# Fatlonder/tinyfusers

Hardware: AMD Instinct MI355X
Metric: unet_denoise_steps_per_sec (higher is better)
Workload: dtype f16; 1 GPU; SD1.5 UNet single denoise step (CFG batch 2 + DDIM update), 64x64x4 latent, 1 image per GPU, fp16 conv/linear, 50-step DDIM schedule; global_batch=1, parallelism=dp1 (batch-sharded, RCCL weight broadcast only, no per-step collective), launch=hipGraph

## Files before the change

### include/tinyfusers_hip.h

```cpp
#ifndef TINYFUSERS_HIP_H
#define TINYFUSERS_HIP_H
#include <stddef.h>
#include <stdint.h>
#ifdef __cplusplus
extern "C" {
#endif

typedef struct tfStream_st* tfStream_t;
typedef struct tfEvent_st* tfEvent_t;
typedef struct tfGraph_st* tfGraph_t;
typedef struct tfComm_st* tfComm_t;
typedef struct tfFunction_st* tfFunction_t;

#define TF_OK 0
#define TF_E_ARG 10001
#define TF_E_UNSUPPORTED 10002
#define TF_E_WORKSPACE 10003
#define TF_E_STATE 10004

#define TF_MEMCPY_H2D 1
#define TF_MEMCPY_D2H 2
#define TF_MEMCPY_D2D 3

int tf_init(int device);
// ... 203 lines not shown
                       void* workspace, size_t workspace_bytes, const void* x3, const void* x4, int C3, int C4, void* gn_partial,
                       size_t gn_partial_bytes, int gn_groups, int* gn_chunks, tfStream_t s);
int tf_conv2d_fused_norm_16(int dtype, void* y, const void* x, const void* x2, const void* w, const void* bias, const void* bias_nc, long long bias_nc_stride,
                            const void* residual, int N, int H, int W, int C1, int C2, int Cout, int R, int S, int stride, int pad, int upsample,
                            void* workspace, size_t workspace_bytes, const void* x3, const void* x4, int C3, int C4, void* gn_partial,
                            size_t gn_partial_bytes, int gn_groups, int* gn_chunks, void* z, const void* z_gamma, const void* z_beta, float z_eps,
                            int z_silu, int* z_written, tfStream_t s);
int tf_conv2d_gn_16(int dtype, void* y, const void* x, const void* x2, const void* w, const void* bias, const void* bias_nc, long long bias_nc_stride,
                    const void* residual, int N, int H, int W, int C1, int C2, int Cout, int R, int S, int stride, int pad, int upsample,
                    void* workspace, size_t workspace_bytes, const void* x3, const void* x4, int C3, int C4, void* gn_partial,
                    size_t gn_partial_bytes, int gn_groups, int* gn_chunks, const void* in_gamma, const void* in_beta, const void* in_partial,
                    int in_chunks, int in_groups1, const void* in_partial2, int in_chunks2, int in_groups2, int in_groups, float in_eps, int in_silu,
                    tfStream_t s);
int tf_linear_16(int dtype, void* y, const void* x, const void* w, const void* bias, const void* residual, int M, int N, int K, int act,
                 void* workspace, size_t workspace_bytes, tfStream_t s);
int tf_ln_fold_weights_16(int dtype, void* w_out, void* bias_out, void* colsum_out_f32, const void* w, const void* bias, const void* gamma, const void* beta,
                          int N, int K, tfStream_t s);
int tf_linear_ln_16(int dtype, void* y, const void* x, const void* w_folded, const void* bias_folded, const void* colsum_f32, const void* residual,
                    int M, int N, int K, int act, float eps, tfStream_t s);
int tf_gemv_16(int dtype, void* y, const void* x, const void* w, const void* bias, int M, int N, int K, int silu_input, tfStream_t s);
int tf_sdpa_16(int dtype, void* o, const void* q, const void* k, const void* v, int B, int NH, int Tq, int Tk, int HS,
               long long q_sb, long long q_sh, long long q_st, long long k_sb, long long k_sh, long long k_st,
               long long v_sb, long long v_sh, long long v_st, long long o_sb, long long o_sh, long long o_st, int causal, tfStream_t s);
int tf_group_norm_apply_16(int dtype, void* y, const void* x, const void* gamma, const void* beta, const void* partial, int chunks,
                           int N, int HW, int C, int G, float eps, int silu, tfStream_t s);
int tf_group_norm_apply_cat_16(int dtype, void* y, const void* x, const void* x2, const void* gamma, const void* beta, const void* partial, int chunks,
                               int groups1, const void* partial2, int chunks2, int groups2, int N, int HW, int C1, int C2, int G, float eps,
                               int silu, tfStream_t s);
int tf_add_16(int dtype, void* y, const void* a, const void* b, long long n, tfStream_t s);

int tf_silu_f16(void* y, const void* x, long long n, tfStream_t s);
int tf_sigmoid_f16(void* y, const void* x, long long n, tfStream_t s);
int tf_gelu_f16(void* y, const void* x, long long n, tfStream_t s);
int tf_quick_gelu_f16(void* y, const void* x, long long n, tfStream_t s);
int tf_embedding_f16(void* out, const void* table, const void* ids, const void* pos, long long n_tokens, int dim, int vocab,
                     int T, tfStream_t s);
int tf_debug_nonfinite(const void* x, long long nbytes, int is_f32, void* flag, tfStream_t s);
int tf_debug_checksum(const void* x, long long nbytes, void* sum, tfStream_t s);
int tf_geglu_f16(void* y, const void* x, int rows, int C, tfStream_t s);
int tf_add_f16(void* y, const void* a, const void* b, long long n, tfStream_t s);
int tf_add_bias_nc_f16(void* y, const void* x, const void* bias_nc, int N, int HW, int C, tfStream_t s);
int tf_upsample2x_nhwc_f16(void* y, const void* x, int N, int H, int W, int C, tfStream_t s);
int tf_concat_channels_f16(void* y, const void* a, const void* b, long long rows, int Ca, int Cb, tfStream_t s);
int tf_im2col_nhwc_f16(void* y, const void* x, int N, int H, int W, int C, int R, int S, int stride, int pad, int Kpad, tfStream_t s);
int tf_im2col_rows_nhwc_f16(void* y, const void* x, int N, int H, int W, int C, int R, int S, int stride, int pad, int Kpad, int ho_begin, int ho_end,
                            tfStream_t s);
// ... 64 lines not shown
```

### tinyfusers_amd/attention/attention.py

```python
import numpy as np

from .. import config
from ..ff.group_norm import GroupNorm
from ..ff.layer_norm import LayerNorm
from ..ff.linear import Linear, fold_layer_norm, linear_f16, linear_ln_f16
from ..ff.nn import FeedForward
from ..native import hip
from ..storage.tensor import DeviceArray, _sh, is_bfloat16
from ..vision.conv2d import Conv2d, _conv
from .sdpa import sdpa_dual_strided, sdpa_strided


def _concat_rows(ws):
    k = ws[0].shape[1]
    n = sum(w.shape[0] for w in ws)
    out = DeviceArray.empty((n, k), ws[0].dtype, "row")
    off = 0
    for w in ws:
        hip.tf_memcpy_async(out.ptr + off, w.ptr, w.nbytes, 3, _sh())
        off += w.nbytes
    return out


class AttnBlock:

    def __init__(self, in_channels, init=True):
        self.norm = GroupNorm(32, in_channels, init=init)
        self.q = Conv2d(in_channels, in_channels, kernel_size=[1, 1], init=init)
        self.k = Conv2d(in_channels, in_channels, kernel_size=[1, 1], init=init)
        self.v = Conv2d(in_channels, in_channels, kernel_size=[1, 1], init=init)
        self.proj_out = Conv2d(in_channels, in_channels, kernel_size=[1, 1], init=init)

    def __call__(self, x):
# ... 21 lines not shown
class CrossAttention:
    def __init__(self, query_dim, context_dim, n_heads, d_head, init=True):
        self.to_q = Linear(query_dim, n_heads * d_head, bias=False, init=init)
        self.to_k = Linear(context_dim, n_heads * d_head, bias=False, init=init)
        self.to_v = Linear(context_dim, n_heads * d_head, bias=False, init=init)
        self.num_heads = n_heads
        self.head_size = d_head
        self.to_out = [Linear(n_heads * d_head, query_dim, init=init)]
        self._fused = None

    def _fused_weights(self, self_attn):
        key = (self.to_q.weight.wkey, self.to_k.weight.wkey, self.to_v.weight.wkey, self_attn)
        if self._fused is None or self._fused[0] != key:
            ws = [self.to_q.weight, self.to_k.weight, self.to_v.weight] if self_attn else [self.to_k.weight, self.to_v.weight]
            self._fused = (key, _concat_rows(ws))
        return self._fused[1]

    def _folded(self, ln, self_attn):
        w = self._fused_weights(True) if self_attn else self.to_q.weight
        key = (w.wkey, ln.weight.wkey, ln.bias.wkey)
        if getattr(self, "_ln_fold", None) is None or self._ln_fold[0] != key:
            self._ln_fold = (key, fold_layer_norm(w, None, ln))
        return self._ln_fold[1]

    def project_kv(self, context):
        return linear_f16(context, self._fused_weights(False))

    def __call__(self, x, context=None, residual=None, kv=None, ln=None, ip=None):
        if ip is not None and context is None and kv is None:
            raise ValueError("CrossAttention: ip= is for cross-attention (context= or kv=), not self-attention")
        b, t, _ = x.shape
        nh, hs = self.num_heads, self.head_size
        c = nh * hs
        from ..ff import fp8
        mx_in = fp8.ATTENTION and ln is not None and fp8.linear_ok(b * t, 3 * c if (context is None and kv is None) else c, x.shape[-1])
        if mx_in:
            if getattr(self, "_cache8", None) is None:
                self._cache8 = {"qkv": {}, "q": {}, "out": {}}
            x8 = fp8.layer_norm_mx(x, ln)
        if context is None and kv is None:
            if mx_in:
                w8, wsc = fp8.pack_weight(self._fused_weights(True), self._cache8["qkv"])
                qkv = fp8.linear_mx(x8, w8, wsc, None)
            elif ln is not None:
                qkv = linear_ln_f16(x, self._folded(ln, True), ln.eps)
            else:
                qkv = linear_f16(x, self._fused_weights(True))
            q, k, v = qkv, qkv.view((b, t, 3 * c), "row", c), qkv.view((b, t, 3 * c), "row", 2 * c)
            tk, qs, ks = t, (t * 3 * c, hs, 3 * c), (t * 3 * c, hs, 3 * c)
        else:
            if mx_in:
                w8, wsc = fp8.pack_weight(self.to_q.weight, self._cache8["q"])
                q = fp8.linear_mx(x8, w8, wsc, None)
            else:
                q = linear_ln_f16(x, self._folded(ln, False), ln.eps) if ln is not None else linear_f16(x, self.to_q.weight)
            if kv is None:
                kv = self.project_kv(context)
            if hasattr(kv, "ld"):
                tk, ld = kv.arr.shape[1], kv.ld
                k = kv.arr.view(kv.arr.shape, "row", kv.off)
                v = kv.arr.view(kv.arr.shape, "row", kv.off + c)
            else:
                tk, ld = kv.shape[1], 2 * c
                k, v = kv, kv.view(kv.shape, "row", c)
            qs, ks = (t * c, hs, c), (tk * ld, hs, ld)
        o = DeviceArray.empty((b, t, c), x.dtype, "row")
        if config.head_merge == "reference_exact":
            os_ = (nh * t * hs, t * hs, hs)
        else:
            os_ = (t * c, hs, c)
        if ip is None:
            sdpa_strided(o, q, k, v, b, nh, t, tk, hs, qs, ks, ks, os_)
        else:
            kv2, scale_ptr = ip
            if kv2.arr.ndim != 3 or kv2.arr.shape[0] != b or kv2.c != c or kv2.off + 2 * c > kv2.ld:
                raise ValueError(f"CrossAttention: ip K|V {kv2.arr.shape} (columns {kv2.off} .. {kv2.off + 2 * c} of {kv2.ld}) does not fit a batch of {b} with {c} channels")
            tk2 = kv2.arr.shape[1]
            k2s = (tk2 * kv2.ld, hs, kv2.ld)
            sdpa_dual_strided(o, q, k, v, kv2.arr.view(kv2.arr.shape, "row", kv2.off), kv2.arr.view(kv2.arr.shape, "row", kv2.off + c), scale_ptr,
                              b, nh, t, tk, tk2, hs, qs, ks, ks, k2s, k2s, os_)
        lo = self.to_out[0]
        if fp8.ATTENTION and fp8.linear_ok(b * t, lo.weight.shape[0], c):
            if getattr(self, "_cache8", None) is None:
                self._cache8 = {"qkv": {}, "q": {}, "out": {}}
            w8, wsc = fp8.pack_weight(lo.weight, self._cache8["out"])
            return fp8.linear_mx(fp8.quantize_mx(o), w8, wsc, lo.bias, residual=residual)
        return lo(o, residual=residual)


class BasicTransformerBlock:
    def __init__(self, dim, context_dim, n_heads, d_head, init=True):
        self.attn1 = CrossAttention(dim, dim, n_heads, d_head, init=init)
        self.ff = FeedForward(dim, init=init)
        self.attn2 = CrossAttention(dim, context_dim, n_heads, d_head, init=init)
# ... 109 lines not shown
```

### tinyfusers_amd/attention/sdpa.py

```python
import numpy as np

from ..native import check, hip, lib
from ..storage.tensor import DeviceArray, _sh, dtag


def sdpa_strided(o, q, k, v, B, NH, Tq, Tk, HS, qs, ks, vs, os_, causal=False):
    assert dtag(q.dtype) == dtag(k.dtype) == dtag(v.dtype) == dtag(o.dtype), "sdpa: q / k / v / o must hold the same 16-bit type"
    hip.tf_sdpa_16(dtag(q.dtype), o.ptr, q.ptr, k.ptr, v.ptr, B, NH, Tq, Tk, HS, *qs, *ks, *vs, *os_, 1 if causal else 0, _sh())
    return o


SDPA_INSTANCES = {1: "generic", 2: "dma16", 3: "dma32", 4: "dma32_w8", 5: "split"}


def sdpa_instance(dtype, B, NH, Tq, Tk, HS, k_st=None, v_st=None, causal=False):
    k_st, v_st = HS if k_st is None else k_st, HS if v_st is None else v_st
    rc = lib.tf_sdpa_instance(dtag(dtype), B, NH, Tq, Tk, HS, k_st, v_st, 1 if causal else 0)
    if rc not in SDPA_INSTANCES:
        check(rc, "tf_sdpa_instance")
    return SDPA_INSTANCES[rc]


def sdpa_dual_strided(o, q, k, v, k2, v2, scale_ptr, B, NH, Tq, Tk, Tk2, HS, qs, ks, vs, k2s, v2s, os_):
    assert dtag(q.dtype) == dtag(k.dtype) == dtag(v.dtype) == dtag(k2.dtype) == dtag(v2.dtype) == dtag(o.dtype), "sdpa_dual: q / k / v / k2 / v2 / o must hold the same 16-bit type"
    hip.tf_sdpa_dual_16(dtag(q.dtype), o.ptr, q.ptr, k.ptr, v.ptr, Tk, k2.ptr, v2.ptr, Tk2, scale_ptr, B, NH, Tq, HS, *qs, *ks, *vs, *k2s, *v2s, *os_, _sh())
    return o


def sdpa_dual_instance(dtype, B, NH, Tq, Tk, Tk2, HS, k_st=None, v_st=None, k2_st=None, v2_st=None):
    st = [HS if s is None else s for s in (k_st, v_st, k2_st, v2_st)]
    rc = lib.tf_sdpa_dual_instance(dtag(dtype), B, NH, Tq, Tk, Tk2, HS, *st)
    if rc not in SDPA_INSTANCES:
        check(rc, "tf_sdpa_dual_instance")
    return SDPA_INSTANCES[rc]


def _is_causal_mask(m, tq, tk):
    m = np.asarray(m)
    if m.shape[-2:] != (tq, tk):
        return False
    m2 = m.reshape(-1, tq, tk)[0]
    tri = np.tril(np.ones((tq, tk), dtype=bool))
    if m.dtype == np.bool_:
        return bool((m2 == tri).all())
    return bool(np.isneginf(m2[~tri]).all() and (m2[tri] == 0).all())


def _additive_mask(attn_mask, B, NH, Tq, Tk):
    m = np.asarray(attn_mask.numpy() if isinstance(attn_mask, DeviceArray) else attn_mask)
    if m.dtype == np.bool_:
        m = np.where(m, np.float32(0.0), np.float32(-np.inf))
    m = m.astype(np.float32)
    if m.ndim < 2 or m.shape[-2:] != (Tq, Tk):
        m = np.broadcast_to(m, (Tq, Tk)) if m.ndim <= 2 else np.broadcast_to(m, m.shape[:-2] + (Tq, Tk))
    if m.ndim > 2 and int(np.prod(m.shape[:-2])) > 1:
        m = np.broadcast_to(m, (B, NH, Tq, Tk)).reshape(B * NH * Tq, Tk)
    else:
# ... 52 lines not shown
```

### tinyfusers_amd/build.py

```python
import concurrent.futures as cf
import os
import subprocess
import sys

HERE = os.path.dirname(os.path.abspath(__file__))
CSRC = os.path.join(HERE, "csrc")
LIBDIR = os.path.join(HERE, "lib")
LIB = os.path.join(LIBDIR, "libtinyfusers_hip.so")
LIB_ABLATION = os.path.join(LIBDIR, "libtinyfusers_hip_ablation.so")
LIB_ASAN = os.path.join(LIBDIR, "libtinyfusers_hip_asan.so")
ASAN_FLAGS = ["-fsanitize=address,undefined", "-fno-gpu-sanitize", "-fno-omit-frame-pointer", "-g", "-fno-sanitize-recover=undefined"]
SOURCES = ["gemm_k_pp16.hip", "gemm_k_pp16_bf16.hip", "gemm_k_pp8.hip", "gemm_k_igemm_128.hip", "gemm_k_igemm_128_bf16.hip", "gemm_k_igemm_64.hip", "gemm_k_igemm_64_bf16.hip",
           "gemm_k_igemm_160.hip", "gemm_k_igemm_160_bf16.hip", "gemm_k_patch.hip", "gemm_k_patch_bf16.hip", "sdpa.hip", "sdpa_bf16.hip", "sdpa_split.hip", "sdpa_split_bf16.hip",
           "sdpa_dual.hip", "sdpa_dual_bf16.hip", "gemm_k_igemm8.hip", "gemm_k_c4.hip", "gemm_k_c4_bf16.hip", "gemm_k_c8.hip", "gemm_k_c8_bf16.hip", "gemm_k_ar.hip", "gemm_k_ar_bf16.hip", "gemm_k_pp3.hip", "gemm_k_pp3_bf16.hip", "gemm.hip", "gemm_reduce.hip", "norm.hip", "elementwise.hip", "runtime.hip", "sgemm.hip",
           "comm.hip", "rtc.hip", "sampler.hip", "img2img.hip", "control.hip", "lora.hip", "vit.hip", "freeu.hip"]
FLAGS = ["--offload-arch=gfx950", "-O3", "-fPIC", "-std=c++17", "-Wall", "-Wno-unused-function", "-ffp-contract=fast"]
SDPA_UNITS = ["sdpa.hip", "sdpa_bf16.hip", "sdpa_split.hip", "sdpa_split_bf16.hip", "sdpa_dual.hip", "sdpa_dual_bf16.hip"]
EXTRA = {s: ["-mllvm", "-amdgpu-mfma-vgpr-form", "-fno-honor-nans"] for s in SDPA_UNITS}


def _hipcc():
    for c in (os.environ.get("HIPCC"), "/opt/rocm/bin/hipcc", "hipcc"):
        if c and (os.path.isabs(c) and os.path.exists(c) or not os.path.isabs(c)):
            return c
    raise RuntimeError("hipcc not found")


def _stale(target, deps):
    if not os.path.exists(target):
        return True
    t = os.path.getmtime(target)
    return any(os.path.getmtime(d) > t for d in deps)


def sanitizer_env(base=None):
    import glob
# ... 40 lines not shown
```

### tinyfusers_amd/config.py

```python
import os


def _flag(name, default):
    v = os.environ.get(name)
    return default if v is None else v not in ("0", "", "false", "False")


head_merge = "reference_exact"

fuse_layer_norm = _flag("TF_FUSE_LAYER_NORM", True)

parallel_branches = _flag("TF_PARALLEL_BRANCHES", False)

fold_skip_projection = _flag("TF_FOLD_SKIP", True)

fold_proj_out = _flag("TF_FOLD_PROJ_OUT", True)

concat_stats = _flag("TF_CONCAT_STATS", True)
concat_stats_max_elems = int(os.environ.get("TF_CONCAT_STATS_MAX_ELEMS", str(4 << 20)))

fuse_group_norm = _flag("TF_FUSE_GROUP_NORM", True)
fuse_group_norm_max_elems = int(os.environ.get("TF_FUSE_GROUP_NORM_MAX_ELEMS", str(4 << 20)))
fuse_group_norm_3x3 = _flag("TF_FUSE_GROUP_NORM_3X3", False)

fuse_reduce_norm = _flag("TF_FUSE_REDUCE_NORM", True)

cfg_parallel = _flag("TF_CFG_PARALLEL", False)

hoist_step_invariants = _flag("TF_HOIST_STEP_INVARIANTS", True)

dtype = "fp16"


def set_dtype(name):
    global dtype
    if name not in ("fp16", "fp8", "bf16"):
        raise ValueError(f"config.set_dtype: unknown dtype {name!r}")
    if name == "bf16" and (parallel_branches or cfg_parallel):
        raise ValueError("config.set_dtype('bf16'): not with TF_PARALLEL_BRANCHES / TF_CFG_PARALLEL (fp16-only experiments)")
# ... 6 lines not shown
```

### tinyfusers_amd/csrc/gemm.hip

```cpp
#include "gemm_prof.h"

__global__ void __launch_bounds__(256) k_quantize_fp8(unsigned char* __restrict__ y, const half_t* __restrict__ x, float scale, long long n8) {
  long long gs = (long long)gridDim.x * 256;
  for (long long i = (long long)blockIdx.x * 256 + threadIdx.x; i < n8; i += gs) {
    h8 v = *reinterpret_cast<const h8*>(x + i * 8);
    f4 a, b;
    for (int e = 0; e < 4; ++e) { a[e] = (float)v[e] * scale; b[e] = (float)v[4 + e] * scale; }
    *reinterpret_cast<uint2*>(y + i * 8) = pack8_fp8(a, b);
  }
}
__global__ void __launch_bounds__(256) k_quantize_mx8(unsigned char* __restrict__ y, const half_t* __restrict__ x, long long rows, int C) {
  const long long n8 = rows * (C >> 3), gs = (long long)gridDim.x * 256;
  const int cv8 = C >> 3;
  for (long long i0 = (long long)blockIdx.x * 256; i0 < n8; i0 += gs) {
    const long long i = i0 + threadIdx.x;
    const bool live = i < n8;
    f4 a = {0.f, 0.f, 0.f, 0.f}, b = {0.f, 0.f, 0.f, 0.f};
    if (live) {
      h8 v = *reinterpret_cast<const h8*>(x + i * 8);
      for (int e = 0; e < 4; ++e) { a[e] = (float)v[e]; b[e] = (float)v[4 + e]; }
    }
    unsigned sb;
    const uint2 code = mx_quant8(a, b, sb);
    if (live) {
// ... 608 lines not shown
int tf_ln_fold_weights_f16(void* w_out, void* bias_out, void* colsum_out, const void* w, const void* bias, const void* gamma, const void* beta,
                           int N, int K, tfStream_t s) {
  return tf_ln_fold_weights_16(TF_DTYPE_F16, w_out, bias_out, colsum_out, w, bias, gamma, beta, N, K, s);
}

int tf_linear_ln_16(int dtype, void* y, const void* x, const void* w_folded, const void* bias_folded, const void* colsum, const void* residual, int M, int N,
                    int K, int act, float eps, tfStream_t s) {
  TF_REQUIRE_DTYPE("tf_linear_ln_16");
  TF_REQUIRE(bias_folded && colsum, "tf_linear_ln_f16: null tensor");
  TF_REQUIRE(K >= 64 && K % 64 == 0, "tf_linear_ln_f16: K=%d must be a positive multiple of 64", K);
  TF_REQUIRE((act == 1 ? N % 16 == 0 : N % 4 == 0), "tf_linear_ln_f16: N=%d must be a multiple of 4 (16 for GEGLU)", N);
  GemmP p;
  int rc = linear_problem(p, "tf_linear_ln_f16", EL_16, y, x, w_folded, bias_folded, residual, M, N, K, act);
  if (rc || M == 0) return rc;
  p.ln_colsum = (const float*)colsum; p.ln_eps = eps;
  p.bf16 = dtype == TF_DTYPE_BF16;
  return run_forced(p, nullptr, 0, s);
}
int tf_linear_ln_f16(void* y, const void* x, const void* w_folded, const void* bias_folded, const void* colsum, const void* residual, int M, int N,
                     int K, int act, float eps, tfStream_t s) {
  return tf_linear_ln_16(TF_DTYPE_F16, y, x, w_folded, bias_folded, colsum, residual, M, N, K, act, eps, s);
}

int tf_gemv_16(int dtype, void* y, const void* x, const void* w, const void* bias, int M, int N, int K, int silu_input, tfStream_t s) {
  TF_REQUIRE_DTYPE("tf_gemv_16");
  TF_REQUIRE(y && x && w && M >= 1 && M <= 8 && N >= 1 && K % 8 == 0, "tf_gemv_f16: needs 1 <= M <= 8 (M=%d) and K %% 8 == 0 (K=%d)", M, K);
  if (dtype == TF_DTYPE_BF16) hipLaunchKernelGGL(k_gemv<true>, dim3(ceil_div(N, 4)), dim3(256), 0, tf_hs(s), (half_t*)y, (const half_t*)x, (const half_t*)w, (const half_t*)bias, M, N, K, silu_input);
  else hipLaunchKernelGGL(k_gemv<false>, dim3(ceil_div(N, 4)), dim3(256), 0, tf_hs(s), (half_t*)y, (const half_t*)x, (const half_t*)w, (const half_t*)bias, M, N, K, silu_input);
  TF_LAUNCH_CHECK();
  return TF_OK;
}
int tf_gemv_f16(void* y, const void* x, const void* w, const void* bias, int M, int N, int K, int silu_input, tfStream_t s) {
  return tf_gemv_16(TF_DTYPE_F16, y, x, w, bias, M, N, K, silu_input, s);
}

}
```

### tinyfusers_amd/csrc/gemm_family.h

```cpp
#pragma once
#include "gemm_reduce.h"

enum Variant {
  V_NONE = -1,
  V_RING = 0,
  V_WIDE = 1,
  V_PATCH = 2,
  V_ALL8 = 3,
  V_PP = 4,
  V_C4 = 5,
  V_PP3 = 6,
  V_C8 = 7,
  V_AR = 8,
  V_COUNT
};
struct TileCfg { int bm, bn, splitk; };

static int g_part16 = 1;
static int g_slab_gm = 1;
static int g_pp_np = 0;

#define TF_GN_MAX_CHUNKS 192
static int gn_reduce_chunks(int HoWo) { int R = (HoWo + TF_GN_MAX_CHUNKS - 1) / TF_GN_MAX_CHUNKS; while (HoWo % R) ++R; return HoWo / R; }
static int gn_pieces(const GemmP& p, int bn) { return bn % p.gn_cpg == 0 ? 1 : 2; }
// ... 47 lines not shown
}
static bool c4_ok(const GemmP& p) {
  if (p.fp8 || p.gi_part || p.gn_part || p.bias_nc || p.out32 || p.out8 || p.on_z) return false;
  if (p.S != 1 || p.stride != 1 || p.pad != 0 || p.ups || p.C3 || p.C4 || p.K != p.Kc) return false;
  if ((p.C1 % 64) || (p.C2 % 64) || (p.N % 8) || p.M < 1) return false;
  return p.act == 0 || (p.act == 1 && p.N % 64 == 0);
}
static bool ar_ok(const GemmP& p) { return c4_ok(p) && (p.K == 256 || p.K == 320) && !p.residual; }

static bool gi_tile_ok(const GemmP& p, int bm, int bn, int variant) {
  if (!p.gi_part) return true;
  if (gemm_generic(p) || p.act || p.ln_colsum || p.HoWo % bm) return false;
  if (p.S == 3) return variant == V_PATCH && patch_admits(p, bm, bn);
  if (p.S != 1 || p.Kc != p.C || p.stride != 1 || p.pad != 0 || p.ups) return false;
  if (variant == V_PATCH || (bm == 128 && bn == 160)) return false;
  return ((igemm_lds_bytes(bm, bn, variant == V_WIDE) + 15) & ~15) + gi_table_bytes(p) <= 163840;
}
static bool gi_any_ok(const GemmP& p) {
  static const int cand[][2] = {{128, 160}, {64, 160}, {128, 128}, {64, 128}, {128, 64}, {64, 64}};
  for (int ci = 0; ci < 6; ++ci)
    for (int v = V_RING; v <= V_ALL8; ++v)
      if (gi_tile_ok(p, cand[ci][0], cand[ci][1], v)) return true;
  return false;
}

#define TF_BF(p, fn, ...) ((p).bf16 ? fn##_bf16(__VA_ARGS__) : fn(__VA_ARGS__))
static bool ring_admits(const GemmP& p, int bm, int bn, int, int variant) { return !(p.bf16 && p.fp8) && !p.mx && gi_tile_ok(p, bm, bn, variant); }
static int ring_launch(GemmP& p, hipStream_t st, int bm, int bn, int variant) {
  const bool wide = variant == V_WIDE, all8 = variant == V_ALL8;
  if (p.fp8) return tfk_launch_igemm8(p, st, bm, bn);
  if (bm == 256 && bn == 128) return TF_BF(p, tfk_launch_igemm_256x128, p, st);
  if (bn == 160) return TF_BF(p, tfk_launch_igemm_160, p, st, bm, wide, all8);
  if (bn == 128) return TF_BF(p, tfk_launch_igemm_128, p, st, bm, wide, all8);
  if (bn == 64) return TF_BF(p, tfk_launch_igemm_64, p, st, bm, wide, all8);
  tf_set_error("run_gemm: no kernel for tile %dx%d", bm, bn);
  return TF_E_UNSUPPORTED;
}
struct Family {
  const char* name;
  bool pingpong;
  bool (*admits)(const GemmP& p, int bm, int bn, int sk, int variant);
  int (*launch)(GemmP& p, hipStream_t st, int bm, int bn, int variant);
  TileCfg (*own_tile)(const GemmP& p);
  bool forced_tile_first;
  int fallback;
  int retile_rows;
// ... 74 lines not shown
```

### tinyfusers_amd/csrc/gemm_igemm.h

```cpp
#pragma once
#include "gemm_common.h"

template <int BM, int BN, bool GENERIC, bool WIDE, bool ALL8 = false, bool GI = false, bool BF = false>
__global__ void __launch_bounds__(512, WIDE ? 4 : 2) k_igemm(const GemmP p) {
  constexpr int TM = BM / 2, TN = BN / 2, MJ = TM / 16, NI = TN / 16;
  constexpr bool EPRE = !WIDE && TF_IGEMM_EPRE;
  constexpr int NG = (BM + BN) / 8;
  constexpr int LPC = ALL8 ? (BN >= 128 ? (BM + BN >= 256 ? 3 : 2) : 1) : 0;
  constexpr int LPS = NG / 4 - LPC;
  static_assert(!(ALL8 && (WIDE || GENERIC)), "ALL8 is a deep-ring, 64-channel-aligned variant");
  static_assert(4 * LPC <= BN / 8, "the consumers take weight groups only");
  constexpr int STAGE = (BM + BN) * 128;
  constexpr int NS = WIDE ? 2 : ring_slots(BM, BN);
  static_assert(NG % 4 == 0 && BM % 32 == 0 && BN % 32 == 0, "tile shape");
  static_assert((NS - 2) * LPS <= 63 || WIDE, "vmcnt immediate is 6 bits");
  extern __shared__ __attribute__((aligned(16))) char smem[];

  const int tid = threadIdx.x;
  const int lane = tid & 63;
  const int wid = __builtin_amdgcn_readfirstlane(tid >> 6);
  const bool loader = wid >= 4;
  const int w4 = wid & 3;
  const int ntiles = p.ntm * p.ntn;
  const int nblk = ntiles * p.splitk;
  const int bid = xcd_order(blockIdx.x, nblk);
  const int split = bid / ntiles;
  const TileMN tmn = tile_decode(bid - split * ntiles, p.order, p.ntm, p.ntn);
// ... 203 lines not shown
      if (ln_on && nt > 0) ln_tile(0);
      asm volatile("" ::: "memory");
      for (int it = 0; it < nt; ++it) {
#if TF_IGEMM_STAMP == 2
        lp(it, 0);
#endif
        if (it + 1 < nt) wait_stages<LPS, NS - 2>(nt - 2 - it);
#if TF_IGEMM_STAMP == 2
        lp(it, 1);
#endif
        if (gi_on && it + 1 < nt) gi_tile((it + 1) % NS, kt_begin + it + 1);
        __builtin_amdgcn_s_barrier();
        asm volatile("" ::: "memory");
#if TF_IGEMM_STAMP == 2
        lp(it, 2);
#endif
        if (it + NS < nt) stage(it % NS, kt_begin + it + NS);
#if TF_IGEMM_STAMP == 2
        lp(it, 3);
#endif
        if (ln_on && it + 1 < nt) ln_tile((it + 1) % NS);
      }
    }
    EpiPre<BM, BN> epre;
    if constexpr (EPRE) igemm_epilogue_prefetch<BM, BN>(p, m0, n0, w4, 1, lane, epre);
    f2 lstat[LPS];
    if (ln_on) {
      const float invK = 1.0f / (float)p.K;
#pragma unroll
      for (int i = 0; i < LPS; ++i) {
        float s_ = ls[i], q_ = lq[i];
#pragma unroll
        for (int o = 1; o < 8; o <<= 1) { s_ += __shfl_xor(s_, o, 64); q_ += __shfl_xor(q_, o, 64); }
        float mean = s_ * invK;
        float var = fmaxf(q_ * invK - mean * mean, 0.f);
        lstat[i] = (f2){mean, rsqrtf(var + p.ln_eps)};
      }
    }
#if TF_IGEMM_STAMP
    IG_STAMP(stp2);
#endif
    __builtin_amdgcn_s_barrier();
    asm volatile("" ::: "memory");
    if (TF_ABL(p.dbg & 1)) return;
    if (ln_on) {
      constexpr int TMl = BM / 2, TNl = BN / 2;
      f2* stats = reinterpret_cast<f2*>(smem + 4 * TMl * (TNl + 4) * 4);
#pragma unroll
      for (int i = 0; i < LPS; ++i) {
        const int g = w4 + 4 * i;
        if (g * 8 < BM && (lane & 7) == 0) stats[8 * g + sub] = lstat[i];
      }
      asm volatile("s_waitcnt lgkmcnt(0)" ::: "memory");
      __builtin_amdgcn_s_barrier();
      asm volatile("" ::: "memory");
    }
    __builtin_amdgcn_s_barrier();
    asm volatile("" ::: "memory");
    igemm_epilogue<BM, BN, false, BF, 4, false, EPRE, true>(p, smem, m0, n0, split, w4, 1, lane, nullptr, 0, 0, epre);
    if (p.gn_part) igemm_gn_stats<BM, BN>(p, smem, m0, n0, w4, 1, lane);
#if TF_IGEMM_STAMP
    asm volatile("s_waitcnt vmcnt(0)" ::: "memory");
    IG_STAMP(stp3);
    if (wid == 4) stamp_out(4);
    lp_out();
#endif
    return;
  }

  if constexpr (GI) gi_prologue<BF>(p, smem, m0 / p.HoWo, w4 * 64 + lane);
  const int wave_m = w4 & 1, wave_n = w4 >> 1;
  const int lr = lane & 15, lg = lane >> 4;
  f4 acc[NI][MJ];
#pragma unroll
  for (int i = 0; i < NI; ++i)
#pragma unroll
    for (int j = 0; j < MJ; ++j) acc[i][j] = (f4){0.f, 0.f, 0.f, 0.f};
  constexpr bool CSUM_LATE = BM == 128 && BN == 160;
  f4 csum[NI];
  auto load_csum = [&]() {
#pragma unroll
    for (int i = 0; i < NI; ++i) {
      int n = n0 + wave_n * TN + i * 16 + lg * 4;
// ... 174 lines not shown
  EpiPre<BM, BN> epre;
  if constexpr (EPRE) igemm_epilogue_prefetch<BM, BN>(p, m0, n0, w4, 0, lane, epre);
  __builtin_amdgcn_s_barrier();
  asm volatile("" ::: "memory");
#if TF_IGEMM_STAMP
  IG_STAMP(stp1);
#endif
  if (TF_ABL(p.dbg & 1)) {
#pragma unroll
    for (int i = 0; i < NI; ++i)
#pragma unroll
      for (int j = 0; j < MJ; ++j) asm volatile("" ::"v"(acc[i][j]));
    return;
  }
  if constexpr (CSUM_LATE) load_csum();
  if (p.ln_colsum) {
    __builtin_amdgcn_s_barrier();
    asm volatile("" ::: "memory");
  }
  igemm_scratch_write<BM, BN>(p, acc, csum, smem, w4, lane);
  asm volatile("s_waitcnt lgkmcnt(0)" ::: "memory");
  __builtin_amdgcn_s_barrier();
  asm volatile("" ::: "memory");
  igemm_epilogue<BM, BN, false, BF, 4, false, EPRE, true>(p, smem, m0, n0, split, w4, 0, lane, nullptr, 0, 0, epre);
  if (p.gn_part) igemm_gn_stats<BM, BN>(p, smem, m0, n0, w4, 0, lane);
#if TF_IGEMM_STAMP
  IG_STAMP(stp2);
  asm volatile("s_waitcnt vmcnt(0)" ::: "memory");
  IG_STAMP(stp3);
  if (wid == 0) stamp_out(0);
  lp_out();
#endif
}
#undef IG_STAMP
```

Measured before the change: 216.9 steps/s.

## Fuse cross-attention Q projection with SDPA in the igemm epilogue

Adds a fused kernel that computes the LayerNorm-folded Q projection with the implicit-GEMM pipeline and then runs cross-attention over the short context (Tk up to 80) directly in the epilogue. K/V tiles are DMA'd into LDS while the GEMM drains, and softmax(QK^T)V is done with MFMA, so Q never goes to global memory and one launch is saved per cross-attention. In exchange it uses a 64x160 tile with a large LDS footprint, which may lower occupancy and tile efficiency compared with the tuned standalone GEMM and SDPA kernels. It is enabled by default for fp16 when the admission checks pass.

```diff
diff --git a/include/tinyfusers_hip.h b/include/tinyfusers_hip.h
--- a/include/tinyfusers_hip.h
+++ b/include/tinyfusers_hip.h
@@ -249,6 +249,11 @@
 int tf_sdpa_16(int dtype, void* o, const void* q, const void* k, const void* v, int B, int NH, int Tq, int Tk, int HS,
                long long q_sb, long long q_sh, long long q_st, long long k_sb, long long k_sh, long long k_st,
                long long v_sb, long long v_sh, long long v_st, long long o_sb, long long o_sh, long long o_st, int causal, tfStream_t s);
+int tf_linear_ln_xattn_16(int dtype, void* o, void* q_out, const void* x, const void* w, const void* bias, const void* colsum_f32, float eps,
+                          const void* k, const void* v, int B, int NH, int Tq, int Tk, int HS, int K, long long k_sb, long long k_sh, long long k_st,
+                          long long v_sb, long long v_sh, long long v_st, long long o_sb, long long o_sh, long long o_st, tfStream_t s);
+int tf_xattn_admits(int dtype, int B, int NH, int Tq, int Tk, int HS, int K, long long k_sb, long long k_sh, long long k_st, long long v_sb, long long v_sh,
+                    long long v_st, long long o_sb, long long o_sh, long long o_st);
 int tf_group_norm_apply_16(int dtype, void* y, const void* x, const void* gamma, const void* beta, const void* partial, int chunks,
                            int N, int HW, int C, int G, float eps, int silu, tfStream_t s);
 int tf_group_norm_apply_cat_16(int dtype, void* y, const void* x, const void* x2, const void* gamma, const void* beta, const void* partial, int chunks,
diff --git a/tinyfusers_amd/attention/attention.py b/tinyfusers_amd/attention/attention.py
--- a/tinyfusers_amd/attention/attention.py
+++ b/tinyfusers_amd/attention/attention.py
@@ -8,7 +8,7 @@
 from ..native import hip
 from ..storage.tensor import DeviceArray, _sh, is_bfloat16
 from ..vision.conv2d import Conv2d, _conv
-from .sdpa import sdpa_dual_strided, sdpa_strided
+from .sdpa import linear_ln_xattn, sdpa_dual_strided, sdpa_strided, xattn_admits
 
 
 def _concat_rows(ws):
@@ -76,6 +76,12 @@
         if getattr(self, "_ln_fold", None) is None or self._ln_fold[0] != key:
             self._ln_fold = (key, fold_layer_norm(w, None, ln))
         return self._ln_fold[1]
+
+    def _os(self, b, t):
+        nh, hs = self.num_heads, self.head_size
+        if config.head_merge == "reference_exact":
+            return (nh * t * hs, t * hs, hs)
+        return (t * nh * hs, hs, nh * hs)
 
     def project_kv(self, context):
         return linear_f16(context, self._fused_weights(False))
@@ -103,11 +109,6 @@
             q, k, v = qkv, qkv.view((b, t, 3 * c), "row", c), qkv.view((b, t, 3 * c), "row", 2 * c)
             tk, qs, ks = t, (t * 3 * c, hs, 3 * c), (t * 3 * c, hs, 3 * c)
         else:
-            if mx_in:
-                w8, wsc = fp8.pack_weight(self.to_q.weight, self._cache8["q"])
-                q = fp8.linear_mx(x8, w8, wsc, None)
-            else:
-                q = linear_ln_f16(x, self._folded(ln, False), ln.eps) if ln is not None else linear_f16(x, self.to_q.weight)
             if kv is None:
                 kv = self.project_kv(context)
             if hasattr(kv, "ld"):
@@ -118,12 +119,22 @@
                 tk, ld = kv.shape[1], 2 * c
                 k, v = kv, kv.view(kv.shape, "row", c)
             qs, ks = (t * c, hs, c), (tk * ld, hs, ld)
+            fused = (config.fuse_cross_attention and ip is None and not mx_in
+                     and not (0 < config.fuse_cross_attention_max_rows < b * t)
+                     and xattn_admits(x.dtype, b, nh, t, tk, hs, x.shape[-1], ks, ks, self._os(b, t)))
+            if fused:
+                q = None
+            elif mx_in:
+                w8, wsc = fp8.pack_weight(self.to_q.weight, self._cache8["q"])
+                q = fp8.linear_mx(x8, w8, wsc, None)
+            else:
+                q = linear_ln_f16(x, self._folded(ln, False), ln.eps) if ln is not None else linear_f16(x, self.to_q.weight)
         o = DeviceArray.empty((b, t, c), x.dtype, "row")
-        if config.head_merge == "reference_exact":
-            os_ = (nh * t * hs, t * hs, hs)
-        else:
-            os_ = (t * c, hs, c)
-        if ip is None:
+        os_ = self._os(b, t)
+        if q is None:
+            linear_ln_xattn(o, x, self._folded(ln, False) if ln is not None else (self.to_q.weight, None, None), ln.eps if ln is not None else 0.0,
+                            k, v, b, nh, t, tk, hs, ks, ks, os_)
+        elif ip is None:
             sdpa_strided(o, q, k, v, b, nh, t, tk, hs, qs, ks, ks, os_)
         else:
             kv2, scale_ptr = ip
diff --git a/tinyfusers_amd/attention/sdpa.py b/tinyfusers_amd/attention/sdpa.py
--- a/tinyfusers_amd/attention/sdpa.py
+++ b/tinyfusers_amd/attention/sdpa.py
@@ -33,6 +33,21 @@
     if rc not in SDPA_INSTANCES:
         check(rc, "tf_sdpa_dual_instance")
     return SDPA_INSTANCES[rc]
+
+
+def xattn_admits(dtype, B, NH, Tq, Tk, HS, K, ks, vs, os_):
+    if not hasattr(lib, "tf_xattn_admits"):
+        return False
+    return lib.tf_xattn_admits(dtag(dtype), B, NH, Tq, Tk, HS, K, *ks, *vs, *os_) == 1
+
+
+def linear_ln_xattn(o, x, folded, eps, k, v, B, NH, Tq, Tk, HS, ks, vs, os_, q_out=None):
+    wf, bf, cs = folded
+    assert dtag(x.dtype) == dtag(k.dtype) == dtag(v.dtype) == dtag(o.dtype) == dtag(wf.dtype), "linear_ln_xattn: x / w / k / v / o must hold the same 16-bit type"
+    hip.tf_linear_ln_xattn_16(dtag(x.dtype), o.ptr, q_out.ptr if q_out is not None else None, x.ptr, wf.ptr, bf.ptr if bf is not None else None,
+                              cs.ptr if cs is not None else None, float(np.asarray(eps).reshape(-1)[0]), k.ptr, v.ptr, B, NH, Tq, Tk, HS, x.shape[-1],
+                              *ks, *vs, *os_, _sh())
+    return o
 
 
 def _is_causal_mask(m, tq, tk):
diff --git a/tinyfusers_amd/build.py b/tinyfusers_amd/build.py
--- a/tinyfusers_amd/build.py
+++ b/tinyfusers_amd/build.py
@@ -11,7 +11,7 @@
 LIB_ASAN = os.path.join(LIBDIR, "libtinyfusers_hip_asan.so")
 ASAN_FLAGS = ["-fsanitize=address,undefined", "-fno-gpu-sanitize", "-fno-omit-frame-pointer", "-g", "-fno-sanitize-recover=undefined"]
 SOURCES = ["gemm_k_pp16.hip", "gemm_k_pp16_bf16.hip", "gemm_k_pp8.hip", "gemm_k_igemm_128.hip", "gemm_k_igemm_128_bf16.hip", "gemm_k_igemm_64.hip", "gemm_k_igemm_64_bf16.hip",
-           "gemm_k_igemm_160.hip", "gemm_k_igemm_160_bf16.hip", "gemm_k_patch.hip", "gemm_k_patch_bf16.hip", "sdpa.hip", "sdpa_bf16.hip", "sdpa_split.hip", "sdpa_split_bf16.hip",
+           "gemm_k_igemm_160.hip", "gemm_k_igemm_160_bf16.hip", "gemm_k_igemm_xattn.hip", "gemm_k_patch.hip", "gemm_k_patch_bf16.hip", "sdpa.hip", "sdpa_bf16.hip", "sdpa_split.hip", "sdpa_split_bf16.hip",
            "sdpa_dual.hip", "sdpa_dual_bf16.hip", "gemm_k_igemm8.hip", "gemm_k_c4.hip", "gemm_k_c4_bf16.hip", "gemm_k_c8.hip", "gemm_k_c8_bf16.hip", "gemm_k_ar.hip", "gemm_k_ar_bf16.hip", "gemm_k_pp3.hip", "gemm_k_pp3_bf16.hip", "gemm.hip", "gemm_reduce.hip", "norm.hip", "elementwise.hip", "runtime.hip", "sgemm.hip",
            "comm.hip", "rtc.hip", "sampler.hip", "img2img.hip", "control.hip", "lora.hip", "vit.hip", "freeu.hip"]
 FLAGS = ["--offload-arch=gfx950", "-O3", "-fPIC", "-std=c++17", "-Wall", "-Wno-unused-function", "-ffp-contract=fast"]
diff --git a/tinyfusers_amd/config.py b/tinyfusers_amd/config.py
--- a/tinyfusers_amd/config.py
+++ b/tinyfusers_amd/config.py
@@ -15,6 +15,9 @@
 fold_skip_projection = _flag("TF_FOLD_SKIP", True)
 
 fold_proj_out = _flag("TF_FOLD_PROJ_OUT", True)
+
+fuse_cross_attention = _flag("TF_FUSE_CROSS_ATTENTION", True)
+fuse_cross_attention_max_rows = int(os.environ.get("TF_FUSE_CROSS_ATTENTION_MAX_ROWS", "8192"))
 
 concat_stats = _flag("TF_CONCAT_STATS", True)
 concat_stats_max_elems = int(os.environ.get("TF_CONCAT_STATS_MAX_ELEMS", str(4 << 20)))
diff --git a/tinyfusers_amd/csrc/gemm.hip b/tinyfusers_amd/csrc/gemm.hip
--- a/tinyfusers_amd/csrc/gemm.hip
+++ b/tinyfusers_amd/csrc/gemm.hip
@@ -654,6 +654,41 @@
   return tf_linear_ln_16(TF_DTYPE_F16, y, x, w_folded, bias_folded, colsum, residual, M, N, K, act, eps, s);
 }
 
+int tf_xattn_admits(int dtype, int B, int NH, int Tq, int Tk, int HS, int K, long long k_sb, long long k_sh, long long k_st, long long v_sb, long long v_sh,
+                    long long v_st, long long o_sb, long long o_sh, long long o_st) {
+  return xattn_admits("tf_xattn_admits", {dtype, B, NH, Tq, Tk, HS, K, k_sb, k_sh, k_st, v_sb, v_sh, v_st, o_sb, o_sh, o_st}) ? 1 : 0;
+}
+int tf_linear_ln_xattn_16(int dtype, void* o, void* q_out, const void* x, const void* w, const void* bias, const void* colsum, float eps, const void* k,
+                          const void* v, int B, int NH, int Tq, int Tk, int HS, int K, long long k_sb, long long k_sh, long long k_st, long long v_sb,
+                          long long v_sh, long long v_st, long long o_sb, long long o_sh, long long o_st, tfStream_t s) {
+  TF_REQUIRE(o && x && w && k && v, "tf_linear_ln_xattn_16: null tensor");
+  if (!xattn_admits("tf_linear_ln_xattn_16", {dtype, B, NH, Tq, Tk, HS, K, k_sb, k_sh, k_st, v_sb, v_sh, v_st, o_sb, o_sh, o_st})) return TF_E_UNSUPPORTED;
+  const uintptr_t al = (uintptr_t)k | (uintptr_t)v | (uintptr_t)x | (uintptr_t)w | (uintptr_t)q_out | (uintptr_t)bias;
+  TF_REQUIRE((al & 15) == 0 && ((uintptr_t)o & 7) == 0, "tf_linear_ln_xattn_16: x / w / bias / k / v / q_out must be 16-byte aligned, o 8-byte aligned");
+  GemmP p;
+  int rc = linear_problem(p, "tf_linear_ln_xattn_16", EL_16, o, x, w, bias, nullptr, B * Tq, NH * HS, K, 0);
+  if (rc) return rc;
+  p.y = (half_t*)q_out;
+  p.ln_colsum = (const float*)colsum; p.ln_eps = eps;
+  const TunedCfg t = {{XA_BM, XA_BN, 1}, V_RING, 0};
+  p.ktiles = K / 64; p.ktiles_per_split = p.ktiles; p.splitk = 1; p.order = t.order;
+  p.ntm = p.M / XA_BM; p.ntn = p.N / XA_BN;
+  fast_div_magic((unsigned)p.HoWo, &p.dv_howo_mul, &p.dv_howo_shr);
+  fast_div_magic((unsigned)p.Wo, &p.dv_wo_mul, &p.dv_wo_shr);
+  XattnP xp;
+  xp.k = (const half_t*)k; xp.v = (const half_t*)v; xp.o = (half_t*)o;
+  xp.Tq = Tq; xp.Tk = Tk; xp.HS = HS;
+  xp.k_sb = k_sb; xp.k_sh = k_sh; xp.k_st = k_st; xp.v_sb = v_sb; xp.v_sh = v_sh; xp.v_st = v_st; xp.o_sb = o_sb; xp.o_sh = o_sh; xp.o_st = o_st;
+  xp.scale_log2e = (1.0f / sqrtf((float)HS)) * 1.4426950408889634f;
+  hipStream_t st = tf_hs(s);
+  ProfRec rec;
+  if (g_prof && (rc = prof_begin(&rec, p, t, st))) return rc;
+  rc = tfk_launch_xattn(p, xp, st);
+  if (g_prof_end) { if (!rc) TF_HIP(hipEventRecord(g_prof_end, st)); g_prof_end = nullptr; }
+  if (g_prof && !rc) tf_prof_fam_add(TF_PROF_FAM_SDPA, 4.0 * B * NH * (double)Tq * Tk * HS, 0.0);
+  return g_prof ? prof_end(&rec, p, t, rc, st) : rc;
+}
+
 int tf_gemv_16(int dtype, void* y, const void* x, const void* w, const void* bias, int M, int N, int K, int silu_input, tfStream_t s) {
   TF_REQUIRE_DTYPE("tf_gemv_16");
   TF_REQUIRE(y && x && w && M >= 1 && M <= 8 && N >= 1 && K % 8 == 0, "tf_gemv_f16: needs 1 <= M <= 8 (M=%d) and K %% 8 == 0 (K=%d)", M, K);
diff --git a/tinyfusers_amd/csrc/gemm_family.h b/tinyfusers_amd/csrc/gemm_family.h
--- a/tinyfusers_amd/csrc/gemm_family.h
+++ b/tinyfusers_amd/csrc/gemm_family.h
@@ -1,5 +1,6 @@
 #pragma once
 #include "gemm_reduce.h"
+#include "gemm_xattn.h"
 
 enum Variant {
   V_NONE = -1,
@@ -93,6 +94,25 @@
     for (int v = V_RING; v <= V_ALL8; ++v)
       if (gi_tile_ok(p, cand[ci][0], cand[ci][1], v)) return true;
   return false;
+}
+
+struct XattnArgs { int dtype, B, NH, Tq, Tk, HS, K; long long k_sb, k_sh, k_st, v_sb, v_sh, v_st, o_sb, o_sh, o_st; };
+static bool xattn_admits(const char* who, const XattnArgs& a) {
+  if (a.dtype != TF_DTYPE_F16) { tf_set_error("%s: dtype=%d: the fused form is float16 only (bfloat16 runs tf_linear_ln_16 + tf_sdpa_16)", who, a.dtype); return false; }
+  if (a.B < 1 || a.NH < 1) { tf_set_error("%s: bad sizes B=%d NH=%d", who, a.B, a.NH); return false; }
+  if (a.HS != 40 && a.HS != 80 && a.HS != 160) { tf_set_error("%s: head size %d: the fused form is built for 40, 80 and 160", who, a.HS); return false; }
+  if ((a.NH * a.HS) % XA_BN) { tf_set_error("%s: NH * HS = %d must be a multiple of %d (whole heads in a %d x %d tile)", who, a.NH * a.HS, XA_BN, XA_BM, XA_BN); return false; }
+  if (a.Tq < XA_BM || a.Tq % XA_BM) { tf_set_error("%s: Tq=%d must be a positive multiple of %d (an m-tile must not span two images)", who, a.Tq, XA_BM); return false; }
+  if (a.Tk < 1 || a.Tk > 80) { tf_set_error("%s: Tk=%d: the epilogue holds 1 .. 80 keys", who, a.Tk); return false; }
+  if (a.K < 64 || a.K % 64) { tf_set_error("%s: K=%d must be a positive multiple of 64", who, a.K); return false; }
+  const long long st8[] = {a.k_sb, a.k_sh, a.k_st, a.v_sb, a.v_sh, a.v_st}, st4[] = {a.o_sb, a.o_sh, a.o_st};
+  for (long long v : st8) if (v < 0 || v % 8) { tf_set_error("%s: k / v strides must be non-negative multiples of 8 elements (16-B rows)", who); return false; }
+  for (long long v : st4) if (v < 0 || v % 4) { tf_set_error("%s: output strides must be non-negative multiples of 4 elements", who); return false; }
+  const long long nht = XA_BN / a.HS;
+  const long long kspan = ((long long)(a.Tk - 1) * a.k_st + (nht - 1) * a.k_sh + a.HS) * 2, vspan = ((long long)(a.Tk - 1) * a.v_st + (nht - 1) * a.v_sh + a.HS) * 2;
+  if (kspan >= (1ll << 31) || vspan >= (1ll << 31)) { tf_set_error("%s: the keys / values of one tile span %lld / %lld bytes; the epilogue addresses them with 32-bit byte offsets", who, kspan, vspan); return false; }
+  if ((long long)a.B * a.Tq >= (1ll << 31)) { tf_set_error("%s: B * Tq = %lld rows is beyond 32-bit indexing", who, (long long)a.B * a.Tq); return false; }
+  return true;
 }
 
 #define TF_BF(p, fn, ...) ((p).bf16 ? fn##_bf16(__VA_ARGS__) : fn(__VA_ARGS__))
diff --git a/tinyfusers_amd/csrc/gemm_igemm.h b/tinyfusers_amd/csrc/gemm_igemm.h
--- a/tinyfusers_amd/csrc/gemm_igemm.h
+++ b/tinyfusers_amd/csrc/gemm_igemm.h
@@ -1,8 +1,21 @@
 #pragma once
 #include "gemm_common.h"
 
+#ifndef TF_IGEMM_XATTN
+#define TF_IGEMM_XATTN 0
+#endif
+#if TF_IGEMM_XATTN
+#define TF_IGEMM_KERNEL k_igemm_xattn
+#define TF_IGEMM_KARGS const GemmP p, const XattnP xp
+#else
+#define TF_IGEMM_KERNEL k_igemm
+#define TF_IGEMM_KARGS const GemmP p
+#endif
 template <int BM, int BN, bool GENERIC, bool WIDE, bool ALL8 = false, bool GI = false, bool BF = false>
-__global__ void __launch_bounds__(512, WIDE ? 4 : 2) k_igemm(const GemmP p) {
+__global__ void __launch_bounds__(512, WIDE ? 4 : 2) TF_IGEMM_KERNEL(TF_IGEMM_KARGS) {
+#if TF_IGEMM_XATTN
+  static_assert(!GENERIC && !WIDE && !GI && !BF && ring_slots(BM, BN) == 5, "the cross-attention epilogue rides on the five-slot deep ring (plain or all-8), fp16");
+#endif
   constexpr int TM = BM / 2, TN = BN / 2, MJ = TM / 16, NI = TN / 16;
   constexpr bool EPRE = !WIDE && TF_IGEMM_EPRE;
   constexpr int NG = (BM + BN) / 8;
@@ -252,6 +265,9 @@
         if (ln_on && it + 1 < nt) ln_tile((it + 1) % NS);
       }
     }
+#if TF_IGEMM_XATTN
+    xattn_issue_kv(xp, smem, m0, n0, w4, lane);
+#endif
     EpiPre<BM, BN> epre;
     if constexpr (EPRE) igemm_epilogue_prefetch<BM, BN>(p, m0, n0, w4, 1, lane, epre);
     f2 lstat[LPS];
@@ -287,8 +303,12 @@
     }
     __builtin_amdgcn_s_barrier();
     asm volatile("" ::: "memory");
+#if TF_IGEMM_XATTN
+    xattn_epilogue<BM, BN>(p, xp, smem, m0, n0, w4, 1, lane, epre);
+#else
     igemm_epilogue<BM, BN, false, BF, 4, false, EPRE, true>(p, smem, m0, n0, split, w4, 1, lane, nullptr, 0, 0, epre);
     if (p.gn_part) igemm_gn_stats<BM, BN>(p, smem, m0, n0, w4, 1, lane);
+#endif
 #if TF_IGEMM_STAMP
     asm volatile("s_waitcnt vmcnt(0)" ::: "memory");
     IG_STAMP(stp3);
@@ -509,8 +529,12 @@
   asm volatile("s_waitcnt lgkmcnt(0)" ::: "memory");
   __builtin_amdgcn_s_barrier();
   asm volatile("" ::: "memory");
+#if TF_IGEMM_XATTN
+  xattn_epilogue<BM, BN>(p, xp, smem, m0, n0, w4, 0, lane, epre);
+#else
   igemm_epilogue<BM, BN, false, BF, 4, false, EPRE, true>(p, smem, m0, n0, split, w4, 0, lane, nullptr, 0, 0, epre);
   if (p.gn_part) igemm_gn_stats<BM, BN>(p, smem, m0, n0, w4, 0, lane);
+#endif
 #if TF_IGEMM_STAMP
   IG_STAMP(stp2);
   asm volatile("s_waitcnt vmcnt(0)" ::: "memory");
@@ -520,3 +544,5 @@
 #endif
 }
 #undef IG_STAMP
+#undef TF_IGEMM_KERNEL
+#undef TF_IGEMM_KARGS
diff --git a/tinyfusers_amd/csrc/gemm_k_igemm_xattn.hip b/tinyfusers_amd/csrc/gemm_k_igemm_xattn.hip
--- /dev/null
+++ b/tinyfusers_amd/csrc/gemm_k_igemm_xattn.hip
@@ -0,0 +1,23 @@
+#define TF_IGEMM_XATTN 1
+#include "gemm_xattn.h"
+#include "gemm_igemm.h"
+#include <stdlib.h>
+#include <string.h>
+
+template <bool ALL8>
+static int launch_xattn(const GemmP& p, const XattnP& xp, hipStream_t st) {
+  constexpr int ring = ring_slots(XA_BM, XA_BN) * (XA_BM + XA_BN) * 128;
+  constexpr int smem = ring > XA_LDS ? ring : XA_LDS;
+  static bool attr_set = false;
+  if (!attr_set) {
+    TF_HIP(hipFuncSetAttribute((const void*)k_igemm_xattn<XA_BM, XA_BN, false, false, ALL8, false, false>, hipFuncAttributeMaxDynamicSharedMemorySize, 163840));
+    attr_set = true;
+  }
+  hipLaunchKernelGGL((k_igemm_xattn<XA_BM, XA_BN, false, false, ALL8, false, false>), dim3(p.ntm * p.ntn), dim3(512), smem, st, p, xp);
+  TF_LAUNCH_CHECK();
+  return TF_OK;
+}
+static const int g_xattn_ring = getenv("TF_XATTN_RING") ? (strcmp(getenv("TF_XATTN_RING"), "plain") == 0 ? 0 : 3) : 3;
+int tfk_launch_xattn(const GemmP& p, const XattnP& xp, hipStream_t st) {
+  return g_xattn_ring == 3 ? launch_xattn<true>(p, xp, st) : launch_xattn<false>(p, xp, st);
+}
diff --git a/tinyfusers_amd/csrc/gemm_xattn.h b/tinyfusers_amd/csrc/gemm_xattn.h
--- /dev/null
+++ b/tinyfusers_amd/csrc/gemm_xattn.h
@@ -0,0 +1,180 @@
+#pragma once
+#include "gemm_common.h"
+
+struct XattnP {
+  const half_t* k; const half_t* v; half_t* o;
+  int Tq, Tk, HS;
+  long long k_sb, k_sh, k_st, v_sb, v_sh, v_st, o_sb, o_sh, o_st;
+  float scale_log2e;
+};
+
+int tfk_launch_xattn(const GemmP& p, const XattnP& xp, hipStream_t st);
+
+constexpr int XA_BM = 64, XA_BN = 160;
+constexpr int XA_KPC = 22, XA_VPC = 21, XA_QPC = 26;
+constexpr int XA_KP = XA_KPC * 8, XA_VP = XA_VPC * 8, XA_QP = XA_QPC * 8;
+constexpr int XA_KROWS = 96;
+constexpr int XA_NKI = XA_KROWS * XA_KPC / 64, XA_NVI = (XA_KROWS * XA_VPC + 63) / 64;
+constexpr int XA_K0 = 45056, XA_V0 = XA_K0 + XA_NKI * 1024, XA_Q0 = XA_V0 + XA_NVI * 1024, XA_LDS = XA_Q0 + XA_BM * XA_QPC * 16;
+static_assert(XA_KROWS * XA_KPC % 64 == 0, "the K image is whole pieces");
+static_assert(XA_K0 >= 4 * (XA_BM / 2) * (XA_BN / 2 + 4) * 4 + XA_BM * 8, "the landing zone lies above the scratch and the (mean, rstd) table");
+static_assert(XA_LDS <= 163840, "LDS of a CU");
+
+__device__ __forceinline__ float xa_max4(float v) {
+  typedef unsigned u2v __attribute__((ext_vector_type(2)));
+  u2v r = __builtin_amdgcn_permlane16_swap(__float_as_uint(v), __float_as_uint(v), false, false);
+  float m = fmaxf(__uint_as_float(r[0]), __uint_as_float(r[1]));
+  u2v q = __builtin_amdgcn_permlane32_swap(__float_as_uint(m), __float_as_uint(m), false, false);
+  return fmaxf(__uint_as_float(q[0]), __uint_as_float(q[1]));
+}
+__device__ __forceinline__ float xa_sum4(float v) {
+  typedef unsigned u2v __attribute__((ext_vector_type(2)));
+  u2v r = __builtin_amdgcn_permlane16_swap(__float_as_uint(v), __float_as_uint(v), false, false);
+  float m = __uint_as_float(r[0]) + __uint_as_float(r[1]);
+  u2v q = __builtin_amdgcn_permlane32_swap(__float_as_uint(m), __float_as_uint(m), false, false);
+  return __uint_as_float(q[0]) + __uint_as_float(q[1]);
+}
+__device__ __forceinline__ s4v xa_tr16(const half_t* p) { return __builtin_amdgcn_ds_read_tr16_b64_v4i16((__attribute__((address_space(3))) s4v*)p); }
+
+__device__ __forceinline__ void xattn_issue_kv(const XattnP& xp, char* smem, int m0, int n0, int w4, int lane) {
+  const int b = m0 / xp.Tq, h0 = n0 / xp.HS, cph = xp.HS >> 3, nht = XA_BN / xp.HS;
+  const unsigned hmul = 256u / (unsigned)cph + 1u;
+  const i4v rs_k = raw_rsrc(xp.k + b * xp.k_sb + h0 * xp.k_sh, (unsigned)(((long long)(xp.Tk - 1) * xp.k_st + (long long)(nht - 1) * xp.k_sh + xp.HS) * 2));
+  const i4v rs_v = raw_rsrc(xp.v + b * xp.v_sb + h0 * xp.v_sh, (unsigned)(((long long)(xp.Tk - 1) * xp.v_st + (long long)(nht - 1) * xp.v_sh + xp.HS) * 2));
+  const unsigned lds_k = lds_off(smem) + XA_K0, lds_v = lds_off(smem) + XA_V0;
+  const int k_st = (int)xp.k_st, k_sh = (int)xp.k_sh, v_st = (int)xp.v_st, v_sh = (int)xp.v_sh;
+#pragma unroll
+  for (int i = 0; i < (XA_NKI + XA_NVI + 3) / 4; ++i) {
+    const int j = w4 + 4 * i;
+    if (j < XA_NKI) {
+      const int x = 64 * j + lane, r = x / XA_KPC, cc = x - r * XA_KPC;
+      const int kt = r >> 4, rr = r & 15;
+      const int key = 32 * (kt >> 1) + 8 * (rr >> 2) + 4 * (kt & 1) + (rr & 3);
+      const int hh = (int)(((unsigned)cc * hmul) >> 8), c = cc - hh * cph;
+      dma16(rs_k, (cc < 20 && key < xp.Tk) ? (unsigned)(key * k_st + hh * k_sh + c * 8) * 2u : TF_OOB, lds_k + (unsigned)j * 1024u);
+    } else if (j < XA_NKI + XA_NVI) {
+      const int x = 64 * (j - XA_NKI) + lane, r = x / XA_VPC, cc = x - r * XA_VPC;
+      const int hh = (int)(((unsigned)cc * hmul) >> 8), c = cc - hh * cph;
+      dma16(rs_v, (cc < 20 && r < xp.Tk) ? (unsigned)(r * v_st + hh * v_sh + c * 8) * 2u : TF_OOB, lds_v + (unsigned)(j - XA_NKI) * 1024u);
+    }
+  }
+}
+
+template <int HS>
+__device__ __forceinline__ void xattn_core(const XattnP& xp, const char* smem, int m0, int n0, int wv, int lane) {
+  constexpr int QT = HS == 40 ? 2 : 1, NKS = (HS + 31) / 32, NDT = (HS + 15) / 16;
+  if (HS == 160 && wv >= 4) return;
+  const int hh = HS == 40 ? wv >> 1 : HS == 80 ? wv >> 2 : 0;
+  const int qt0 = HS == 40 ? (wv & 1) * 2 : (wv & 3);
+  const int lr = lane & 15, lg = lane >> 4;
+  const half_t* qs = reinterpret_cast<const half_t*>(smem + XA_Q0) + hh * HS;
+  const half_t* ks = reinterpret_cast<const half_t*>(smem + XA_K0) + hh * HS;
+  const half_t* vs = reinterpret_cast<const half_t*>(smem + XA_V0) + hh * HS;
+  const f4 zero4 = {0.f, 0.f, 0.f, 0.f};
+  h8 qf[QT][NKS];
+#pragma unroll
+  for (int qt = 0; qt < QT; ++qt)
+#pragma unroll
+    for (int s_ = 0; s_ < NKS; ++s_) {
+      const int d0 = s_ * 32 + lg * 8;
+      qf[qt][s_] = d0 < HS ? *reinterpret_cast<const h8*>(qs + ((qt0 + qt) * 16 + lr) * XA_QP + d0) : (h8){0, 0, 0, 0, 0, 0, 0, 0};
+    }
+  f4 st[6][QT];
+#pragma unroll
+  for (int kt = 0; kt < 6; ++kt)
+#pragma unroll
+    for (int s_ = 0; s_ < NKS; ++s_) {
+      const h8 kf = *reinterpret_cast<const h8*>(ks + (16 * kt + lr) * XA_KP + s_ * 32 + lg * 8);
+#pragma unroll
+      for (int qt = 0; qt < QT; ++qt) st[kt][qt] = mfma16<false>(kf, qf[qt][s_], s_ == 0 ? zero4 : st[kt][qt]);
+    }
+  h8 pf[3][QT];
+  float inv[QT];
+#pragma unroll
+  for (int qt = 0; qt < QT; ++qt) {
+    float m = -INFINITY;
+#pragma unroll
+    for (int kt = 0; kt < 6; ++kt)
+#pragma unroll
+      for (int e = 0; e < 4; ++e) {
+        const int key = 32 * (kt >> 1) + 8 * lg + 4 * (kt & 1) + e;
+        if (key >= xp.Tk) st[kt][qt][e] = -INFINITY;
+        m = fmaxf(m, st[kt][qt][e]);
+      }
+    m = xa_max4(m);
+    float l = 0.f;
+#pragma unroll
+    for (int kt = 0; kt < 6; ++kt)
+#pragma unroll
+      for (int e = 0; e < 4; ++e) {
+        const half_t pr = (half_t)__builtin_amdgcn_exp2f(st[kt][qt][e] - m);
+        pf[kt >> 1][qt][(kt & 1) * 4 + e] = pr;
+        l += (float)pr;
+      }
+    l = xa_sum4(l);
+    inv[qt] = l > 0.f ? 1.0f / l : 0.f;
+  }
+  f4 ot[NDT][QT];
+#pragma unroll
+  for (int dt = 0; dt < NDT; ++dt)
+#pragma unroll
+    for (int qt = 0; qt < QT; ++qt) ot[dt][qt] = zero4;
+#pragma unroll
+  for (int dt = 0; dt < NDT; ++dt)
+#pragma unroll
+    for (int kc = 0; kc < 3; ++kc) {
+      const half_t* va = vs + (32 * kc + 8 * lg + (lr >> 2)) * XA_VP + dt * 16 + 4 * (lr & 3);
+      union { struct { s4v a, b; } s; h8 h; } u;
+      u.s.a = xa_tr16(va); u.s.b = xa_tr16(va + 4 * XA_VP);
+#pragma unroll
+      for (int qt = 0; qt < QT; ++qt) ot[dt][qt] = mfma16<false>(u.h, pf[kc][qt], ot[dt][qt]);
+    }
+  const int b = m0 / xp.Tq, t0 = m0 - b * xp.Tq;
+  half_t* ob = xp.o + b * xp.o_sb + (n0 / HS + hh) * xp.o_sh;
+#pragma unroll
+  for (int qt = 0; qt < QT; ++qt) {
+    const long long qi = t0 + (qt0 + qt) * 16 + lr;
+#pragma unroll
+    for (int dt = 0; dt < NDT; ++dt) {
+      const int d = dt * 16 + lg * 4;
+      if (d < HS) {
+        h4 o;
+#pragma unroll
+        for (int e = 0; e < 4; ++e) o[e] = (half_t)(ot[dt][qt][e] * inv[qt]);
+        *reinterpret_cast<h4*>(ob + qi * xp.o_st + d) = o;
+      }
+    }
+  }
+}
+
+template <int BM, int BN>
+__device__ __forceinline__ void xattn_epilogue(const GemmP& p, const XattnP& xp, char* smem, int m0, int n0, int w4, int half, int lane, const EpiPre<BM, BN, 4>& pre) {
+  static_assert(BM == XA_BM && BN == XA_BN, "the 64 x 160 tile");
+  constexpr int TM = BM / 2, TN = BN / 2, RS = TN + 4, ROWS = TM / 2, CPR = TN / 8, ITEMS = ROWS * CPR, KB = EpiPre<BM, BN, 4>::KB;
+  static_assert(KB * 64 >= ITEMS, "every item's bias was prefetched");
+  const float* sc = reinterpret_cast<const float*>(smem) + (size_t)w4 * (TM * RS) + (size_t)half * ROWS * RS;
+  const int rb = (w4 & 1) * TM + half * ROWS, cb = (w4 >> 1) * TN;
+  half_t* qs = reinterpret_cast<half_t*>(smem + XA_Q0);
+#pragma unroll
+  for (int k = 0; k < KB; ++k) {
+    const int idx = lane + 64 * k;
+    if (idx >= ITEMS) continue;
+    const int row = idx / CPR, c8 = idx - row * CPR;
+    const float* r = sc + row * RS + c8 * 8;
+    f4 v0 = *reinterpret_cast<const f4*>(r), v1 = *reinterpret_cast<const f4*>(r + 4);
+    if (p.bias) { for (int e = 0; e < 4; ++e) { v0[e] += (float)pre.bv[k][e]; v1[e] += (float)pre.bv[k][4 + e]; } }
+    h8 out, qv;
+    for (int e = 0; e < 4; ++e) { out[e] = (half_t)v0[e]; out[4 + e] = (half_t)v1[e]; }
+    if (p.y) *reinterpret_cast<h8*>(p.y + (long long)(m0 + rb + row) * p.N + n0 + cb + c8 * 8) = out;
+    for (int e = 0; e < 8; ++e) qv[e] = (half_t)((float)out[e] * xp.scale_log2e);
+    *reinterpret_cast<h8*>(qs + (rb + row) * XA_QP + cb + c8 * 8) = qv;
+  }
+  if (half) asm volatile("s_waitcnt vmcnt(0)" ::: "memory");
+  asm volatile("s_waitcnt lgkmcnt(0)" ::: "memory");
+  __builtin_amdgcn_s_barrier();
+  asm volatile("" ::: "memory");
+  const int wv = w4 + 4 * half;
+  if (xp.HS == 40) xattn_core<40>(xp, smem, m0, n0, wv, lane);
+  else if (xp.HS == 80) xattn_core<80>(xp, smem, m0, n0, wv, lane);
+  else xattn_core<160>(xp, smem, m0, n0, wv, lane);
+}
```

After: 218.7 steps/s, median of 6. Within noise of the previous version (+0.8%).
